# dsshim0125/s2p

Measured on AMD Instinct MI355X. Metric: G+D train-step images/sec at 84x84 bs=64/GPU, higher is better.
Workload: dtype bf16; 1 GPU; configs[2]: full G+D train step (hinge GAN + feature matching + VGG19 perceptual + L1, Adam x2), 84x84 cheetah, netG=s2p, netD=multiscale(2); global_batch=64, per_gpu_batch=64, parallelism=dp1, hip_graph=True, graph_segments=1, streams=overlapped, vgg_weights=seeded stand-in (ImageNet weights unobtainable offline)

## Files before the change

include/s2p_hip.h:

```cpp
#ifndef S2P_HIP_H
#define S2P_HIP_H
#include <stddef.h>
#include <stdint.h>

#ifdef __cplusplus
extern "C" {
#endif
#pragma GCC visibility push(default)

#define S2P_VERSION 125

enum { S2P_F32 = 0, S2P_BF16 = 1 };
enum { S2P_ACT_NONE = 0, S2P_ACT_RELU = 1, S2P_ACT_LRELU = 2, S2P_ACT_TANH = 3, S2P_ACT_SWISH = 4 };
enum { S2P_EPI_STORE = 0,
       S2P_EPI_ADD = 1,
       S2P_EPI_MUL_ACTGRAD = 2   };

typedef struct {
  int32_t dtype;
  int32_t N, H, W, Cin, x_pitch;
  int32_t Ho, Wo, Cout, y_pitch;
  int32_t KH, KW, stride, pad;
  int32_t transposed;
  int32_t reflect;
  int32_t groups;
  int32_t x_gstride, y_gstride;
  int32_t cin_real;
} s2p_conv_desc;

int s2p_version(void);
const char* s2p_last_error(void);

int s2p_conv2d_fwd(const s2p_conv_desc* d, const void* x, const void* w_fwd, const float* bias,
                   const void* aux, void* y, int act, float slope, int epi, void* stream);
int s2p_conv2d_dgrad(const s2p_conv_desc* d, const void* dy, const void* w_bwd,
                     const void* aux, const void* aux2, void* dx, int epi, int aux_act, float slope,
                     void* stream);
size_t s2p_conv2d_fwd_workspace(const s2p_conv_desc* d, int epi);
int s2p_conv2d_fwd_ws(const s2p_conv_desc* d, const void* x, const void* w_fwd, const float* bias,
                      const void* aux, void* y, int act, float slope, int epi, void* workspace,
                      size_t workspace_bytes, void* stream);
size_t s2p_conv2d_dgrad_workspace(const s2p_conv_desc* d);
int s2p_conv2d_dgrad_ws(const s2p_conv_desc* d, const void* dy, const void* w_bwd,
                        const void* aux, const void* aux2, void* dx, int epi, int aux_act, float slope,
                        void* workspace, size_t workspace_bytes, void* stream);
int s2p_conv2d_fwd_mat(const s2p_conv_desc* d, const void* x, const void* w_fwd, const float* bias, const void* aux,
                       void* y, int epi, const void* gb_img, int gb_pitch, const float* gb_st, int gb_st_pitch,
                       int act, float slope, float eps, void* y_mat, int y_mat_pitch, float* stats, void* workspace,
                       size_t workspace_bytes, void* stream);
int s2p_conv2d_dgrad_mat(const s2p_conv_desc* d, const void* dy, const void* w_bwd, void* d_mid, const void* aux, const void* xn,
                         int xn_pitch, const float* stats, const void* gb_img, int gb_pitch, const float* gb_st,
                         int gb_st_pitch, int act, float slope, float eps, float* sums, void* dxn, int dxn_pitch,
                         void* dgb_img, int dgb_pitch, float* dgb_st, int dgb_st_pitch, const void* res, int res_pitch,
                         void* workspace, size_t workspace_bytes, void* stream);
int s2p_conv2d_mat_is_fused(const s2p_conv_desc* d, int dgrad, int has_gb);
enum { S2P_CONV_PATH_THIN = 0, S2P_CONV_PATH_THIN4 = 1, S2P_CONV_PATH_THIN_CIN = 2, S2P_CONV_PATH_THIN_ROWS = 3,
       S2P_CONV_PATH_PLANE = 4, S2P_CONV_PATH_PLANEG = 5, S2P_CONV_PATH_HALO = 6, S2P_CONV_PATH_SPLITK = 7,
       S2P_CONV_PATH_DMA = 8, S2P_CONV_PATH_PHASES = 9, S2P_CONV_PATH_GENERIC = 10 };
enum { S2P_HALO_S9_176_PIPE = 0, S2P_HALO_S9_176 = 1, S2P_HALO_S9_320 = 2, S2P_HALO_R_176 = 3, S2P_HALO_R_320 = 4 };
int s2p_conv2d_path(const s2p_conv_desc* d, int dgrad, int has_workspace);
int s2p_conv2d_wgrad(const s2p_conv_desc* d, const void* x, const void* dy, float* dw, float* db,
                     int cin_real, int cout_real, int64_t dw_gstride, int splitk, void* stream);
size_t s2p_conv2d_wgrad_workspace(const s2p_conv_desc* d, int cin_real, int cout_real);
int s2p_conv2d_wgrad_ws(const s2p_conv_desc* d, const void* x, const void* dy, float* dw, float* db,
                        int cin_real, int cout_real, int64_t dw_gstride, int splitk, void* workspace,
                        size_t workspace_bytes, void* stream);
size_t s2p_conv2d_wgrad_det_workspace(const s2p_conv_desc* d, int cin_real, int cout_real, int splitk);
typedef struct { const void* x; const void* dy; float* dw; float* db; } s2p_wgrad_job;
size_t s2p_conv2d_wgrad_batched_workspace(const s2p_conv_desc* d, int n_jobs, int cin_real, int cout_real);
int s2p_conv2d_wgrad_batched(const s2p_conv_desc* d, const s2p_wgrad_job* jobs, int n_jobs, int cin_real,
                             int cout_real, void* workspace, size_t workspace_bytes, void* stream);
int s2p_reflect_pad_bwd(int dtype, const void* dxp, int N, int H, int W, int C, int pad, void* dx,
                        void* stream);
int s2p_channel_sum(int dtype, const void* dy, int64_t pixels, int C, int pitch, float* db,
                    void* stream);
size_t s2p_channel_sum_workspace(int64_t pixels, int C);
int s2p_channel_sum_ws(int dtype, const void* dy, int64_t pixels, int C, int pitch, float* db, void* workspace,
                       size_t workspace_bytes, void* stream);

int64_t s2p_in_stats_floats(int N, int HW, int C);
int s2p_in_stats(int dtype, const void* x, int N, int HW, int C, int pitch, float eps,
                 float* stats, void* stream);
int s2p_in_apply_fwd(int dtype, const void* x, int N, int HW, int C, int pitch,
                     const float* stats, const void* gb_img, int gb_pitch,
                     const float* gb_st, int gb_st_pitch, int act, float slope, float eps,
                     void* y, int y_pitch, void* stream);
int s2p_in_norm_fwd(int dtype, const void* x, int N, int HW, int C, int pitch, const void* gb_img, int gb_pitch,
                    const float* gb_st, int gb_st_pitch, int act, float slope, float eps, void* y, int y_pitch,
                    float* stats, void* stream);
int64_t s2p_in_bwd_sums_floats(int N, int HW, int C);
int s2p_in_bwd_reduce(int dtype, const void* da, int da_pitch, const void* x, int N, int HW, int C,
                      int pitch, const float* stats, const void* gb_img, int gb_pitch,
                      const float* gb_st, int gb_st_pitch, int act, float slope, float eps,
                      float* sums, void* stream);
int s2p_in_bwd_apply(int dtype, const void* da, int da_pitch, const void* x, int N, int HW, int C,
                     int pitch, const float* stats, const void* gb_img, int gb_pitch,
                     const float* gb_st, int gb_st_pitch, int act, float slope, float eps,
                     const float* sums, void* dx, int dx_pitch, void* dgb_img, int dgb_pitch,
                     float* dgb_st, int dgb_st_pitch, void* stream);

int s2p_posenc_fwd(const float* state, int N, int S, int L, float* out, int out_pitch, void* stream);

int s2p_in_norm_bwd(int dtype, const void* da, int da_pitch, const void* x, int N, int HW, int C, int pitch,
                    const float* stats, const void* gb_img, int gb_pitch, const float* gb_st, int gb_st_pitch,
                    int act, float slope, float eps, float* sums, void* dx, int dx_pitch, void* dgb_img,
                    int dgb_pitch, float* dgb_st, int dgb_st_pitch, void* stream);
int s2p_in_norm_bwd_res(int dtype, const void* da, int da_pitch, const void* x, int N, int HW, int C, int pitch,
                        const float* stats, const void* gb_img, int gb_pitch, const float* gb_st, int gb_st_pitch,
                        int act, float slope, float eps, float* sums, void* dx, int dx_pitch, void* dgb_img,
                        int dgb_pitch, float* dgb_st, int dgb_st_pitch, const void* res, int res_pitch, void* stream);

// ... 114 lines not shown
```

s2p_amd/_lib.py:

```python
import ctypes
import os
import subprocess

import torch

_HERE = os.path.dirname(os.path.abspath(__file__))
_SO = os.path.join(_HERE, "csrc", "libs2p_hip.so")

F32, BF16 = 0, 1
ACT_NONE, ACT_RELU, ACT_LRELU, ACT_TANH, ACT_SWISH = 0, 1, 2, 3, 4
EPI_STORE, EPI_ADD, EPI_MUL_ACTGRAD = 0, 1, 2
(PATH_THIN, PATH_THIN4, PATH_THIN_CIN, PATH_THIN_ROWS, PATH_PLANE, PATH_PLANEG, PATH_HALO, PATH_SPLITK, PATH_DMA, PATH_PHASES,
 PATH_GENERIC) = range(11)
HALO_S9_176_PIPE, HALO_S9_176, HALO_S9_320, HALO_R_176, HALO_R_320 = range(5)

c_int, c_float, c_void_p, c_int64 = ctypes.c_int, ctypes.c_float, ctypes.c_void_p, ctypes.c_int64


class ConvDesc(ctypes.Structure):
    _fields_ = [(n, ctypes.c_int32) for n in (
        "dtype", "N", "H", "W", "Cin", "x_pitch", "Ho", "Wo", "Cout", "y_pitch",
        "KH", "KW", "stride", "pad", "transposed", "reflect", "groups", "x_gstride", "y_gstride", "cin_real")]


class L1Job(ctypes.Structure):
    _fields_ = [("a", c_void_p), ("b", c_void_p), ("grad_a", c_void_p), ("count", c_int64), ("scale", c_float),
                ("loss_out", c_void_p)]


class WgradJob(ctypes.Structure):
    _fields_ = [("x", c_void_p), ("dy", c_void_p), ("dw", c_void_p), ("db", c_void_p)]


class PackJob(ctypes.Structure):
    _fields_ = [("src", c_void_p), ("dst_fwd", c_void_p), ("dst_bwd", c_void_p),
                ("R", ctypes.c_int32), ("T", ctypes.c_int32), ("C", ctypes.c_int32),
                ("Cpad", ctypes.c_int32), ("Rrow", ctypes.c_int32), ("r_off", ctypes.c_int32),
                ("dtype", ctypes.c_int32)]


class SnJob(ctypes.Structure):
    _fields_ = [("w", c_void_p), ("u", c_void_p), ("v", c_void_p), ("sigma", c_void_p), ("ws", c_void_p), ("grad", c_void_p),
                ("R", ctypes.c_int32), ("K", ctypes.c_int32)]


_P = c_void_p
_DESC = ctypes.POINTER(ConvDesc)
SIGNATURES = {
    "s2p_version": [],
    "s2p_last_error": [],
    "s2p_conv2d_fwd": [_DESC, _P, _P, _P, _P, _P, c_int, c_float, c_int, _P],
    "s2p_conv2d_dgrad": [_DESC, _P, _P, _P, _P, _P, c_int, c_int, c_float, _P],
    "s2p_conv2d_fwd_workspace": [_DESC, c_int],
    "s2p_conv2d_fwd_ws": [_DESC, _P, _P, _P, _P, _P, c_int, c_float, c_int, _P, ctypes.c_size_t, _P],
    "s2p_conv2d_fwd_mat": [_DESC, _P, _P, _P, _P, _P, c_int, _P, c_int, _P, c_int, c_int, c_float, c_float, _P, c_int, _P, _P,
                           ctypes.c_size_t, _P],
    "s2p_conv2d_dgrad_mat": [_DESC, _P, _P, _P, _P, _P, c_int, _P, _P, c_int, _P, c_int, c_int, c_float, c_float, _P, _P, c_int, _P, c_int,
                             _P, c_int, _P, c_int, _P, ctypes.c_size_t, _P],
    "s2p_conv2d_mat_is_fused": [_DESC, c_int, c_int],
    "s2p_conv2d_path": [_DESC, c_int, c_int],
    "s2p_conv2d_dgrad_workspace": [_DESC],
    "s2p_conv2d_dgrad_ws": [_DESC, _P, _P, _P, _P, _P, c_int, c_int, c_float, _P, ctypes.c_size_t, _P],
    "s2p_conv2d_wgrad": [_DESC, _P, _P, _P, _P, c_int, c_int, c_int64, c_int, _P],
    "s2p_conv2d_wgrad_workspace": [_DESC, c_int, c_int],
    "s2p_conv2d_wgrad_det_workspace": [_DESC, c_int, c_int, c_int],
    "s2p_channel_sum_workspace": [c_int64, c_int],
# ... 136 lines not shown
```

s2p_amd/csrc/conv_igemm.hip:

```cpp
#include "s2p_common.h"
#include "conv_plane.h"
#include "conv_planeg.h"
#include <type_traits>
#include <vector>

#define MAX_TAPS 64

constexpr int PHASE_TAPS = 16, MAX_PHASES = 4;
struct GatherArgs {
  const void* x; const void* w; const float* bias; const void* aux; const void* aux2; void* y;
  int M, Hi, Wi, Qh, Qw;
  int Cin, x_pitch, x_gstride;
  int Cout, Cst, y_pitch, y_gstride;
  int Ho, Wo;
  int istride, ostride, oy0, ox0;
  int T, Ktot, w_row;
  long long w_gstride;
  int reflect, act, epi, gact;
  float slope, gslope;
  int npix_tiles, nco_tiles;
  int halo_lo, halo_hi;
  int diag;
  int splitk, ksteps;
  float* part; int psplit, psteps, part_m;
  void* ws; size_t ws_bytes;
  unsigned x_bytes, w_bytes;
  int tap[MAX_TAPS];
  int nphase, phase_fast;
  struct Phase { int Qh, Qw, M, oy0, ox0, T, Ktot, npix_tiles; int tap[PHASE_TAPS]; } ph[MAX_PHASES];
};

template <typename T> struct Mma;
template <> struct Mma<__bf16> { static constexpr int BK = 32; };
template <> struct Mma<float> { static constexpr int BK = 16; };

template <typename T, int BCO, int BPIX, int TCO, int TPIX>
__device__ __forceinline__ void conv_epilogue(const GatherArgs& a, f32x16 (&acc)[TCO][TPIX], char* smem, const int* rowoff,
                                              int g, int co_base, int wco0, int wpix0, int r, int h, int tid) {
  constexpr int CE = DT<T>::CE;
  constexpr int ERS = BCO * (int)sizeof(T) + 16;
  const float* bias = (a.bias && (blockIdx.z == 0 || a.nphase > 0)) ? a.bias + (size_t)g * a.Cout : nullptr;
  const bool act_generic = (a.act == S2P_ACT_TANH || a.act == S2P_ACT_SWISH);
  const float ns = a.act == S2P_ACT_RELU ? 0.f : (a.act == S2P_ACT_LRELU ? a.slope : 1.f);
  if (bias) {
    const __amdgpu_buffer_rsrc_t brs = __builtin_amdgcn_make_buffer_rsrc((void*)bias, 0, a.Cout * 4, 0x00020000);
#pragma unroll
    for (int i = 0; i < TCO; ++i)
#pragma unroll
      for (int q4 = 0; q4 < 4; ++q4) {
        const int co = co_base + wco0 + 32 * i + 8 * q4 + 4 * h;
        float bv[4];
#pragma unroll
        for (int e = 0; e < 4; ++e) bv[e] = __builtin_bit_cast(float, __builtin_amdgcn_raw_buffer_load_b32(brs, co * 4, e * 4, 0));
#pragma unroll
        for (int j = 0; j < TPIX; ++j)
// ... 500 lines not shown
    if (m >= a.M) break;
    Chunk<T> c;
    float wv[8];
#pragma unroll
    for (int e = 0; e < 8; ++e) {
      const float t = v[e][i];
      float w = lrelu_ns(t, ns);
      if (act_generic) w = a.act == S2P_ACT_TANH ? tanhf(t) : t / (1.f + expf(-t));
      wv[e] = w;
    }
    c.pack(wv);
    const size_t go = (size_t)m * a.y_pitch + co0;
    if (a.epi != S2P_EPI_STORE) {
      Chunk<T> x, x2;
      x.raw = (u32x4){0u, 0u, 0u, 0u}; x2.raw = (u32x4){0u, 0u, 0u, 0u};
      if (full) {
        x.raw = *(const u32x4*)(aux + go);
        if (aux2) x2.raw = *(const u32x4*)(aux2 + go);
      } else {
        for (int e = 0; e < 8; ++e) if (co0 + e < a.Cst) {
          x.set(e, to_f32(aux[go + e]));
          if (aux2) x2.set(e, to_f32(aux2[go + e]));
        }
      }
#pragma unroll
      for (int e = 0; e < 8; ++e) {
        const float xv = x.get(e);
        const float f = g_tanh ? 1.f - xv * xv : (xv > 0.f ? 1.f : gneg);
        wv[e] = epi_add ? c.get(e) + xv : (c.get(e) + x2.get(e)) * f;
      }
      c.pack(wv);
    }
    if (full) *(u32x4*)(y + go) = c.raw;
    else for (int e = 0; e < 8; ++e) if (co0 + e < a.Cst) y[go + e] = from_f32<T>(c.get(e));
  }
}

struct ConvSwitches {
  int no_dma = s2p_env_set("S2P_NO_LDS_DMA");
  int diag = s2p_env_int("S2P_DIAG", 0);
  int no_halo = s2p_env_set("S2P_NO_HALO");
  int no_split = s2p_env_set("S2P_NO_CONV_SPLITK");
  int split_min_steps = s2p_env_int("S2P_SPLIT_MIN_STEPS", 16);
  int split_max_wg = s2p_env_int("S2P_SPLIT_MAX_WG", 160);
  int no_plane = s2p_env_set("S2P_NO_PLANE");
  int halo_extra_lds = s2p_env_int("S2P_HALO_EXTRA_LDS", 0);
  int no_static_taps = s2p_env_set("S2P_NO_STATIC_TAPS");
  int halo_pipe = s2p_env_set("S2P_NO_HALO_PIPE") ? 0 : 1;
  int no_merge = s2p_env_set("S2P_NO_PHASE_MERGE") || s2p_env_set("S2P_NO_LDS_DMA");
  int no_thin_cin = s2p_env_set("S2P_NO_THIN_CIN");
  static bool no_planeg() { return S2P_DIAG_SWITCH(0); }
  static bool no_planeg_3x3() { return S2P_DIAG_SWITCH(2); }
  static bool no_thin4() { return S2P_DIAG_SWITCH(3); }
  static bool no_phase_fast() { return S2P_DIAG_SWITCH(10); }
};
static const ConvSwitches& conv_switches() { static const ConvSwitches sw; return sw; }

static int conv_split_plan(int nwg, int nk) {
  const int min_steps = conv_switches().split_min_steps, max_wg = conv_switches().split_max_wg;
  if (nwg > max_wg || nk < 2 * min_steps) return 1;
  int S = 384 / nwg;
  if (S > nk / min_steps) S = nk / min_steps;
  if (S > 16) S = 16;
  return S < 2 ? 1 : S;
}

template <int NPOS_CAP, bool DBUF>
struct HaloTile {
  static constexpr int BCO = 128, BPIX = 128, WPIX = 2, TCO = 2, TPIX = 2;
  static constexpr int BK = 64, RS = 128;
  static constexpr int WSTAGE = BCO * RS;
  static constexpr int HALO = (NPOS_CAP + 1) * RS;
  static constexpr int ERS = BCO * 2 + 16, EPI = BPIX * ERS;
  static constexpr int NHB = DBUF ? 2 : 1;
  static constexpr int MAIN0 = NHB * HALO + 2 * WSTAGE + 1024;
  static constexpr int MAIN = MAIN0 > EPI ? MAIN0 : EPI;
  static constexpr int NHP = (NPOS_CAP / 8 + 3) / 4;

  char* hbase; char* wbase; char* zrow; int* rowoff;
  int tid, lane, wave, r, h, g, lrow, pc;
  int co_base, pix_base, wco0, wpix0, swr, npos, nslab;
  unsigned w_byte[4], h_byte[NHP];
  unsigned long long vmask[TPIX];
  __amdgpu_buffer_rsrc_t xr, wr;

  __device__ __forceinline__ void setup(const GatherArgs& a, char* smem) {
    rowoff = (int*)(smem + MAIN);
    hbase = smem; wbase = smem + NHB * HALO; zrow = smem + NHB * HALO + 2 * WSTAGE;
    tid = threadIdx.x; lane = tid & 63; r = lane & 31; h = lane >> 5; g = blockIdx.y;
    wave = __builtin_amdgcn_readfirstlane(tid >> 6);
    tile_of_block<BCO, BPIX>(blockIdx.x, a.npix_tiles * a.nco_tiles, a.nco_tiles, co_base, pix_base);
    if (tid < BPIX) rowoff[tid] = pix_base + tid < a.M ? pix_base + tid : -1;
    if (tid < 64) *(u32x4*)(zrow + tid * 16) = (u32x4){0u, 0u, 0u, 0u};
    if (tid < 8 * NHB) *(u32x4*)(hbase + (tid >> 3) * HALO + NPOS_CAP * RS + (tid & 7) * 16) = (u32x4){0u, 0u, 0u, 0u};
    xr = conv_x_rsrc(a, g); wr = conv_w_rsrc(a, g);

    lrow = lane >> 3; pc = lane & 7;
#pragma unroll
    for (int i = 0; i < 4; ++i) w_byte[i] = w_row_dma_byte(a, co_base, (4 * i + wave) * 8 + lrow, pc);
    npos = BPIX + a.halo_lo + a.halo_hi;
#pragma unroll
    for (int i = 0; i < NHP; ++i) h_byte[i] = halo_dma_byte(a, (4 * i + wave) * 8 + lrow);
    wco0 = (wave / WPIX) * (TCO * 32);
    wpix0 = (wave % WPIX) * (TPIX * 32);
    const PixelSplit split(a.Qh, a.Qw);
#pragma unroll
// ... 252 lines not shown
  constexpr bool PIPELINED = TS > 0 && PIPE && DBUF;
  __shared__ __attribute__((aligned(1024))) char smem[HT::MAIN + HT::BPIX * 4];
  unsigned long long tl0 = 0, tl1 = 0, tl2 = 0, st_c0 = 0, st_r0 = 0;
  if (S2P_DIAGV(a) == 9) tl0 = __builtin_amdgcn_s_memrealtime();
  HT t;
  t.setup(a, smem);
  f32x16 acc[HT::TCO][HT::TPIX];
  clear_acc(acc);
  if (S2P_DIAGV(a) == 5) return;
  auto loop_start = [&]() {
    if (S2P_DIAGV(a) == 3) return false;
    if (S2P_DIAGV(a) == 8) { st_c0 = __builtin_amdgcn_s_memtime(); st_r0 = __builtin_amdgcn_s_memrealtime(); }
    if (PIPELINED && S2P_DIAGV(a) == 9) tl1 = __builtin_amdgcn_s_memrealtime();
    return true;
  };
  bool done;
  if constexpr (TS > 0) {
    const HaloStaticTaps<TS> tp(a, t);
    if constexpr (PIPELINED) done = halo_loop_pipelined(a, t, tp, acc, loop_start);
    else done = halo_loop_static(a, t, tp, acc, loop_start);
  } else {
    done = halo_loop_runtime(a, t, acc, loop_start);
  }
  if (!done) return;
  if (S2P_DIAGV(a) == 8) {
    const unsigned long long c1 = __builtin_amdgcn_s_memtime(), r1 = __builtin_amdgcn_s_memrealtime();
    if (t.tid == 0 && t.g == 0) {
      unsigned long long* o = (unsigned long long*)a.y + (size_t)blockIdx.x * 2;
      o[0] = c1 - st_c0; o[1] = r1 - st_r0;
    }
    if (acc[0][0][0] == 12345.678f) ((float*)a.y)[7] = acc[1][1][3] + acc[0][1][2] + acc[1][0][1];
    return;
  }
  if constexpr (PIPELINED) {
    asm volatile("s_waitcnt lgkmcnt(0)" ::: "memory");
    __syncthreads();
  }
  if (S2P_DIAGV(a) == 4) { if (acc[0][0][0] == 12345.678f) ((float*)a.y)[0] = acc[1][1][3] + acc[0][1][2] + acc[1][0][1]; return; }
  if (PIPELINED && S2P_DIAGV(a) == 9) {
    tl2 = __builtin_amdgcn_s_memrealtime();
    GatherArgs b = a; b.aux = nullptr;
    conv_epilogue<__bf16, HT::BCO, HT::BPIX, HT::TCO, HT::TPIX>(b, acc, smem, t.rowoff, t.g, t.co_base, t.wco0, t.wpix0, t.r, t.h, t.tid);
    asm volatile("s_waitcnt vmcnt(0)" ::: "memory");
    __syncthreads();
    if (t.tid == 0 && t.g == 0 && a.aux) {
      unsigned long long* o = (unsigned long long*)a.aux + (size_t)blockIdx.x * 4;
      o[0] = tl0; o[1] = tl1; o[2] = tl2; o[3] = __builtin_amdgcn_s_memrealtime();
    }
    return;
  }
  conv_epilogue<__bf16, HT::BCO, HT::BPIX, HT::TCO, HT::TPIX>(a, acc, smem, t.rowoff, t.g, t.co_base, t.wco0, t.wpix0, t.r, t.h, t.tid);
}

enum class ConvPath { Thin, Thin4, ThinCin, ThinRows, Plane, PlaneG, Halo, SplitK, Dma, Phases, Generic };
static_assert((int)ConvPath::Halo == S2P_CONV_PATH_HALO && (int)ConvPath::Generic == S2P_CONV_PATH_GENERIC, "ids of s2p_conv2d_path");
enum class HaloKind { S9_176_PIPE, S9_176, S9_320, R_176, R_320 };

struct ConvOperands {
  const void* x; const void* w; const float* bias; const void* aux; const void* aux2; void* y;
  int act; float slope; int epi, gact; float gslope;
};
struct NormWant { bool any, gb, bwd; };
struct ScratchAvail { bool any; size_t bytes; };
static const ScratchAvail SCRATCH_UNLIMITED{true, ~(size_t)0};
struct Scratch { void* ws; size_t bytes; };

struct GatherChoice {
  ConvPath path = ConvPath::Generic;
  bool fused = false;
  size_t ws_bytes = 0;
  int bco = 128;
  HaloKind halo = HaloKind::R_320;
  PlaneArgs plane;
  PlaneGArgs planeg;
};
struct GatherItem { GatherArgs a; GatherChoice c; };
struct ConvPlan {
  ConvPath path = ConvPath::Generic;
  bool fused = false;
  size_t ws_bytes = 0;
  int cout_pad = 0;
  std::vector<GatherItem> items;
  void add(const GatherItem& it) {
    if (items.empty()) path = it.c.path;
    if (it.c.ws_bytes > ws_bytes) ws_bytes = it.c.ws_bytes;
    items.push_back(it);
    fused = items.size() == 1 && it.c.fused;
  }
};

template <typename P>
static void copy_conv_fields(P& p, const GatherArgs& a) {
  p.x = a.x; p.w = a.w; p.bias = a.bias; p.aux = a.aux; p.aux2 = a.aux2; p.y = a.y;
  p.Cin = a.Cin; p.x_pitch = a.x_pitch; p.x_gstride = a.x_gstride;
  p.Cout = a.Cout; p.Cst = a.Cst; p.y_pitch = a.y_pitch; p.y_gstride = a.y_gstride;
  p.w_row = a.w_row; p.w_gstride = a.w_gstride;
  p.act = a.act; p.epi = a.epi; p.gact = a.gact; p.slope = a.slope; p.gslope = a.gslope;
  p.x_bytes = a.x_bytes; p.w_bytes = a.w_bytes;
}

static void plan_fast(GatherArgs& a, GatherChoice& c, int groups, const NormWant& want, const ScratchAvail& sc) {
  const ConvSwitches& sw = conv_switches();
  a.npix_tiles = cdiv(a.M, 128);
  a.nco_tiles = cdiv(a.Cst, c.bco);
  a.diag = sw.diag;
  const int nwg = a.npix_tiles * a.nco_tiles;
  const bool whole = a.ostride == 1 && a.oy0 == 0 && a.ox0 == 0 && a.Qh == a.Ho && a.Qw == a.Wo;
  const bool planes = whole && a.M % (a.Qh * a.Qw) == 0;
  int S = 1;
  if (!sw.no_split && groups == 1 && whole && sc.any) S = conv_split_plan(nwg, a.Ktot / 64);
  if (!sw.no_plane && a.T == 9 && a.istride == 1 && planes && a.Qh == a.Hi && a.Qw == a.Wi) {
    PlaneArgs& p = c.plane;
    bool ok = true;
    for (int t = 0; t < 9; ++t) p.wt[t] = -1;
    for (int t = 0; t < 9 && ok; ++t) {
      const int dy = (int)(signed char)(a.tap[t] & 0xff), dx = (int)(signed char)((a.tap[t] >> 8) & 0xff);
      if (dy < -1 || dy > 1 || dx < -1 || dx > 1 || p.wt[(dy + 1) * 3 + dx + 1] >= 0) ok = false;
      else p.wt[(dy + 1) * 3 + dx + 1] = a.tap[t] >> 16;
    }
    copy_conv_fields(p, a);
    p.N = a.M / (a.Qh * a.Qw); p.H = a.Qh; p.W = a.Qw;
    if (ok && s2p_conv_plane_applicable(p)) {
      c.path = ConvPath::Plane;
      c.fused = want.any && groups == 1 && a.act == S2P_ACT_NONE && a.epi != S2P_EPI_MUL_ACTGRAD && (!want.bwd || a.epi == S2P_EPI_STORE);
      return;
    }
  }
  if (!sw.no_plane && !sw.no_planeg() && !(a.T == 9 && sw.no_planeg_3x3()) && groups == 1 && planes && !a.reflect) {
    PlaneGProblem pr{a.M / (a.Qh * a.Qw), a.Hi, a.Wi, a.Ho, a.Wo, a.Cin, a.Cout, a.Cst, a.x_pitch, a.y_pitch, a.istride, a.T, a.tap, want.any};
    PlaneGArgs& p = c.planeg;
    if (s2p_conv_planeg_setup(pr, p)) {
      copy_conv_fields(p, a);
      p.N = pr.N;
      c.path = ConvPath::PlaneG;
      c.fused = want.any && p.nbands == 1 && p.gimg == 1 && !want.gb && a.act == S2P_ACT_NONE && a.epi != S2P_EPI_MUL_ACTGRAD;
      return;
    }
  }
  if (c.bco == 128 && S <= 1 && !sw.no_halo && a.istride == 1 && a.ostride == 1 && a.Qh == a.Hi && a.Qw == a.Wi &&
      a.Ho == a.Qh && a.Wo == a.Qw && a.T >= 4) {
    int lo = 0, hi = 0;
    for (int t = 0; t < a.T; ++t) {
      int off = (int)(signed char)(a.tap[t] & 0xff) * a.Wi + (int)(signed char)((a.tap[t] >> 8) & 0xff);
      if (-off > lo) lo = -off;
      if (off > hi) hi = off;
    }
    const int npos = 128 + lo + hi;
    const bool s9 = a.T == 9 && !sw.no_static_taps;
    if (npos <= 320) {
      a.halo_lo = lo; a.halo_hi = hi;
      c.path = ConvPath::Halo;
      if (npos <= 176) c.halo = s9 ? (sw.halo_pipe && a.Cin % 64 == 0 ? HaloKind::S9_176_PIPE : HaloKind::S9_176) : HaloKind::R_176;
      else c.halo = s9 ? HaloKind::S9_320 : HaloKind::R_320;
      return;
    }
  }
  if (S > 1) {
    const int nk = a.Ktot / 64;
    a.psteps = cdiv(nk, S); a.psplit = cdiv(nk, a.psteps);
    a.part_m = a.npix_tiles * 128;
    const size_t need = (size_t)a.psplit * a.Cst * a.part_m * sizeof(float);
    if (a.psplit > 1 && need <= sc.bytes) { c.path = ConvPath::SplitK; c.ws_bytes = need; return; }
    a.psplit = 1;
  }
  c.path = ConvPath::Dma;
}

static GatherItem plan_gather(const GatherArgs& a_in, bool bf16, int groups, long long x_elems, const NormWant& want, const ScratchAvail& sc) {
  GatherItem it{a_in, {}};
  GatherArgs& a = it.a;
  const long long xb = x_elems * 2, wb = (long long)a.Cout * a.w_row * 2;
  if (bf16 && a.Cin % 64 == 0 && !a.reflect && a.T > 0 && xb < (1ll << 31) && wb < (1ll << 31) && a.Cst > 32 && !conv_switches().no_dma) {
    a.x_bytes = (unsigned)xb; a.w_bytes = (unsigned)wb;
    it.c.bco = a.Cst > 64 ? 128 : 64;
    plan_fast(a, it.c, groups, want, sc);
  }
  return it;
}

static int pack_tap(int dy, int dx, int wt) { return (wt << 16) | ((dx & 0xff) << 8) | (dy & 0xff); }

struct Geo {
  int N, Hi, Wi, Ci, xp, xg, Ho, Wo, Co, Cst, yp, yg, KH, KW, stride, pad, reflect, groups;
  long long w_gstride; int w_row;
// ... 147 lines not shown
  return plan_scatter_problem(G, d->dtype == S2P_BF16, op, want, sc, P);
}

template <int BCO>
static int launch_bf16(GatherArgs& a, const GatherChoice& c, int groups, void* ws, hipStream_t st) {
  const int extra_lds = conv_switches().halo_extra_lds;
  dim3 grid(a.npix_tiles * a.nco_tiles, groups);
  switch (c.path) {
    case ConvPath::Halo:
      if constexpr (BCO == 128) {
        switch (c.halo) {
          case HaloKind::S9_176_PIPE: hipLaunchKernelGGL((conv_halo_kernel<176, true, 9, true>), grid, dim3(256), extra_lds, st, a); break;
          case HaloKind::S9_176: hipLaunchKernelGGL((conv_halo_kernel<176, true, 9>), grid, dim3(256), extra_lds, st, a); break;
          case HaloKind::S9_320: hipLaunchKernelGGL((conv_halo_kernel<320, false, 9>), grid, dim3(256), 0, st, a); break;
          case HaloKind::R_176: hipLaunchKernelGGL((conv_halo_kernel<176, true>), grid, dim3(256), extra_lds, st, a); break;
          case HaloKind::R_320: hipLaunchKernelGGL((conv_halo_kernel<320, false>), grid, dim3(256), 0, st, a); break;
        }
        S2P_CHECK_LAUNCH("conv_halo_kernel");
      }
      return 0;
    case ConvPath::SplitK: {
      a.part = (float*)ws;
      grid.z = a.psplit;
      hipLaunchKernelGGL((conv_dma_kernel<BCO, 128, 2, 2>), grid, dim3(256), 0, st, a);
      S2P_CHECK_LAUNCH("conv_dma_kernel(split)");
      const long long n = (long long)(a.part_m / 4) * ((a.Cst + 7) / 8);
      hipLaunchKernelGGL(conv_part_reduce_kernel, dim3(cdiv(n, 64)), dim3(64), 0, st, a);
      S2P_CHECK_LAUNCH("conv_part_reduce_kernel");
      return 0;
    }
    default:
      hipLaunchKernelGGL((conv_dma_kernel<BCO, 128, 2, 2>), grid, dim3(256), 0, st, a);
      S2P_CHECK_LAUNCH("conv_dma_kernel");
      return 0;
  }
}

template <typename T>
static int launch_generic(GatherArgs& a, int groups, hipStream_t st) {
  if (a.Cst > 64) return launch_cfg<T, 128, 128, 2, 2>(a, groups, st);
  if (a.Cst > 32) return launch_cfg<T, 64, 128, 2, 2>(a, groups, st);
  return launch_cfg<T, 32, 256, 1, 4>(a, groups, st);
}

static int launch_item(GatherItem& it, bool bf16, int groups, const PlaneNorm* mat, void* ws, hipStream_t st) {
  if (!bf16) return launch_generic<float>(it.a, groups, st);
  switch (it.c.path) {
    case ConvPath::Plane:
      if (it.c.fused) it.c.plane.nm = *mat;
      return s2p_conv_plane_launch(it.c.plane, groups, st);
    case ConvPath::PlaneG:
      if (it.c.fused) it.c.planeg.nm = *mat;
      return s2p_conv_planeg_launch(it.c.planeg, groups, st);
    case ConvPath::Phases: {
      GatherArgs& a = it.a;
      int max_npt = 0;
      for (int i = 0; i < a.nphase; ++i) if (a.ph[i].npix_tiles > max_npt) max_npt = a.ph[i].npix_tiles;
      const dim3 grid = a.phase_fast ? dim3(((max_npt * a.nco_tiles + 7) / 8) * 8 * a.nphase, groups, 1) : dim3(max_npt * a.nco_tiles, groups, a.nphase);
      if (it.c.bco == 128) hipLaunchKernelGGL((conv_dma_kernel<128, 128, 2, 2>), grid, dim3(256), 0, st, a);
      else hipLaunchKernelGGL((conv_dma_kernel<64, 128, 2, 2>), grid, dim3(256), 0, st, a);
      S2P_CHECK_LAUNCH("conv_dma_kernel(phases)");
      return 0;
    }
    case ConvPath::Generic: break;
    default: return it.c.bco == 128 ? launch_bf16<128>(it.a, it.c, groups, ws, st) : launch_bf16<64>(it.a, it.c, groups, ws, st);
  }
  return launch_generic<__bf16>(it.a, groups, st);
}
static int launch_items(ConvPlan& P, bool bf16, int groups, const PlaneNorm* mat, const Scratch& sc, hipStream_t st) {
  for (GatherItem& it : P.items) {
    const int rc = launch_item(it, bf16, groups, mat, sc.ws, st);
    if (rc) return rc;
  }
  return 0;
}

static int conv_fwd_impl(const s2p_conv_desc* d, const ConvOperands& op, const PlaneNorm* mat, bool* fused, const Scratch& sc, void* stream) {
  S2P_CHECK_SLOPE("s2p_conv2d_fwd", op.act, op.slope);
  if (mat) S2P_CHECK_SLOPE("s2p_conv2d_fwd_mat", mat->n_act, mat->n_slope);
  ConvPlan P;
  int rc = conv_plan_fwd(d, op, NormWant{mat != nullptr, mat && mat->gb, false}, ScratchAvail{sc.ws != nullptr, sc.bytes}, P);
  if (rc) return rc;
  if (!op.x || !op.w || (!op.y && !mat)) S2P_FAIL(-1, "s2p_conv2d_fwd: null pointer");
  if (op.epi != S2P_EPI_STORE && !op.aux) S2P_FAIL(-1, "s2p_conv2d_fwd: epi needs aux");
  if (!op.y && !P.fused) S2P_FAIL(-1, "s2p_conv2d_fwd_mat: y == NULL needs the fused launch (s2p_conv2d_mat_is_fused)");
  if (fused) *fused = P.fused;
  hipStream_t st = (hipStream_t)stream;
  switch (P.path) {
    case ConvPath::Thin: return s2p_thin_fwd(d, op.x, op.w, op.bias, op.y, op.act, op.slope, st);
    case ConvPath::Thin4: return s2p_thin4_fwd(d, op.x, op.w, op.bias, op.y, op.act, op.slope, sc.ws, sc.bytes, st);
    case ConvPath::ThinCin: return s2p_thin_cin_fwd(d, op.x, op.w, op.bias, op.y, op.act, op.slope, st);
    default: return launch_items(P, d->dtype == S2P_BF16, d->groups, mat, sc, st);
  }
}

extern "C" int s2p_conv2d_fwd(const s2p_conv_desc* d, const void* x, const void* w_fwd, const float* bias,
                              const void* aux, void* y, int act, float slope, int epi, void* stream) {
  return conv_fwd_impl(d, ConvOperands{x, w_fwd, bias, aux, nullptr, y, act, slope, epi, 0, 0.f}, nullptr, nullptr, Scratch{nullptr, 0}, stream);
}
extern "C" int s2p_conv2d_fwd_ws(const s2p_conv_desc* d, const void* x, const void* w_fwd, const float* bias,
                                 const void* aux, void* y, int act, float slope, int epi, void* workspace,
                                 size_t workspace_bytes, void* stream) {
  return conv_fwd_impl(d, ConvOperands{x, w_fwd, bias, aux, nullptr, y, act, slope, epi, 0, 0.f}, nullptr, nullptr,
                       Scratch{workspace, workspace_bytes}, stream);
}
extern "C" int s2p_conv2d_fwd_mat(const s2p_conv_desc* d, const void* x, const void* w_fwd, const float* bias, const void* aux,
// ... 95 lines not shown
```

Before: 7649 images/sec.

## Add persistent streaming 3x3 conv kernel with LDS ring buffer for Cin=64

Adds a new conv path for 3x3 stride-1 convolutions with 64 input channels that would otherwise take the multi-band PlaneG path without fused norm. Each workgroup is persistent per CU and per 64-channel output slice. It keeps all 9 taps of weights resident in LDS and streams input pixels through a padded-row ring buffer, refilling the next tile inside the MFMA K loop. This is meant to remove the repeated weight and halo reloads of the banded PlaneG kernel and to overlap loads with compute. The trade-off is one workgroup per CU at 256 threads, which lowers occupancy and may leave CUs idle when there are few tiles.

```diff
diff --git a/include/s2p_hip.h b/include/s2p_hip.h
--- a/include/s2p_hip.h
+++ b/include/s2p_hip.h
@@ -56,7 +56,7 @@
 int s2p_conv2d_mat_is_fused(const s2p_conv_desc* d, int dgrad, int has_gb);
 enum { S2P_CONV_PATH_THIN = 0, S2P_CONV_PATH_THIN4 = 1, S2P_CONV_PATH_THIN_CIN = 2, S2P_CONV_PATH_THIN_ROWS = 3,
        S2P_CONV_PATH_PLANE = 4, S2P_CONV_PATH_PLANEG = 5, S2P_CONV_PATH_HALO = 6, S2P_CONV_PATH_SPLITK = 7,
-       S2P_CONV_PATH_DMA = 8, S2P_CONV_PATH_PHASES = 9, S2P_CONV_PATH_GENERIC = 10 };
+       S2P_CONV_PATH_DMA = 8, S2P_CONV_PATH_PHASES = 9, S2P_CONV_PATH_GENERIC = 10, S2P_CONV_PATH_STREAM = 11 };
 enum { S2P_HALO_S9_176_PIPE = 0, S2P_HALO_S9_176 = 1, S2P_HALO_S9_320 = 2, S2P_HALO_R_176 = 3, S2P_HALO_R_320 = 4 };
 int s2p_conv2d_path(const s2p_conv_desc* d, int dgrad, int has_workspace);
 int s2p_conv2d_wgrad(const s2p_conv_desc* d, const void* x, const void* dy, float* dw, float* db,
diff --git a/s2p_amd/_lib.py b/s2p_amd/_lib.py
--- a/s2p_amd/_lib.py
+++ b/s2p_amd/_lib.py
@@ -11,7 +11,7 @@
 ACT_NONE, ACT_RELU, ACT_LRELU, ACT_TANH, ACT_SWISH = 0, 1, 2, 3, 4
 EPI_STORE, EPI_ADD, EPI_MUL_ACTGRAD = 0, 1, 2
 (PATH_THIN, PATH_THIN4, PATH_THIN_CIN, PATH_THIN_ROWS, PATH_PLANE, PATH_PLANEG, PATH_HALO, PATH_SPLITK, PATH_DMA, PATH_PHASES,
- PATH_GENERIC) = range(11)
+ PATH_GENERIC, PATH_STREAM) = range(12)
 HALO_S9_176_PIPE, HALO_S9_176, HALO_S9_320, HALO_R_176, HALO_R_320 = range(5)
 
 c_int, c_float, c_void_p, c_int64 = ctypes.c_int, ctypes.c_float, ctypes.c_void_p, ctypes.c_int64
diff --git a/s2p_amd/csrc/conv_igemm.hip b/s2p_amd/csrc/conv_igemm.hip
--- a/s2p_amd/csrc/conv_igemm.hip
+++ b/s2p_amd/csrc/conv_igemm.hip
@@ -1,6 +1,7 @@
 #include "s2p_common.h"
 #include "conv_plane.h"
 #include "conv_planeg.h"
+#include "conv_stream.h"
 #include <type_traits>
 #include <vector>
 
@@ -607,6 +608,7 @@
   static bool no_planeg() { return S2P_DIAG_SWITCH(0); }
   static bool no_planeg_3x3() { return S2P_DIAG_SWITCH(2); }
   static bool no_thin4() { return S2P_DIAG_SWITCH(3); }
+  static bool no_stream() { return S2P_DIAG_SWITCH(21); }
   static bool no_phase_fast() { return S2P_DIAG_SWITCH(10); }
 };
 static const ConvSwitches& conv_switches() { static const ConvSwitches sw; return sw; }
@@ -965,8 +967,9 @@
   conv_epilogue<__bf16, HT::BCO, HT::BPIX, HT::TCO, HT::TPIX>(a, acc, smem, t.rowoff, t.g, t.co_base, t.wco0, t.wpix0, t.r, t.h, t.tid);
 }
 
-enum class ConvPath { Thin, Thin4, ThinCin, ThinRows, Plane, PlaneG, Halo, SplitK, Dma, Phases, Generic };
-static_assert((int)ConvPath::Halo == S2P_CONV_PATH_HALO && (int)ConvPath::Generic == S2P_CONV_PATH_GENERIC, "ids of s2p_conv2d_path");
+enum class ConvPath { Thin, Thin4, ThinCin, ThinRows, Plane, PlaneG, Halo, SplitK, Dma, Phases, Generic, Stream };
+static_assert((int)ConvPath::Halo == S2P_CONV_PATH_HALO && (int)ConvPath::Generic == S2P_CONV_PATH_GENERIC && (int)ConvPath::Stream == S2P_CONV_PATH_STREAM,
+              "ids of s2p_conv2d_path");
 enum class HaloKind { S9_176_PIPE, S9_176, S9_320, R_176, R_320 };
 
 struct ConvOperands {
@@ -986,6 +989,7 @@
   HaloKind halo = HaloKind::R_320;
   PlaneArgs plane;
   PlaneGArgs planeg;
+  StreamArgs stream;
 };
 struct GatherItem { GatherArgs a; GatherChoice c; };
 struct ConvPlan {
@@ -1043,6 +1047,18 @@
     PlaneGProblem pr{a.M / (a.Qh * a.Qw), a.Hi, a.Wi, a.Ho, a.Wo, a.Cin, a.Cout, a.Cst, a.x_pitch, a.y_pitch, a.istride, a.T, a.tap, want.any};
     PlaneGArgs& p = c.planeg;
     if (s2p_conv_planeg_setup(pr, p)) {
+      if (p.nbands > 1 && a.Cin == 64 && !want.any && !sw.no_stream()) {
+        const StreamProblem sp{pr.N, a.Hi, a.Wi, a.Ho, a.Wo, a.Cin, a.Cout, a.Cst, a.x_pitch, a.y_pitch, a.istride, a.T, a.tap};
+        StreamArgs& s = c.stream;
+        if (s2p_conv_stream_setup(sp, s)) {
+          s.x = a.x; s.w = a.w; s.bias = a.bias; s.aux = a.aux; s.aux2 = a.aux2; s.y = a.y;
+          s.x_pitch = a.x_pitch; s.Cout = a.Cout; s.y_pitch = a.y_pitch; s.w_row = a.w_row;
+          s.act = a.act; s.epi = a.epi; s.gact = a.gact; s.slope = a.slope; s.gslope = a.gslope;
+          s.x_bytes = a.x_bytes; s.w_bytes = a.w_bytes;
+          c.path = ConvPath::Stream;
+          return;
+        }
+      }
       copy_conv_fields(p, a);
       p.N = pr.N;
       c.path = ConvPath::PlaneG;
@@ -1296,6 +1312,8 @@
     case ConvPath::PlaneG:
       if (it.c.fused) it.c.planeg.nm = *mat;
       return s2p_conv_planeg_launch(it.c.planeg, groups, st);
+    case ConvPath::Stream:
+      return s2p_conv_stream_launch(it.c.stream, st);
     case ConvPath::Phases: {
       GatherArgs& a = it.a;
       int max_npt = 0;
diff --git a/s2p_amd/csrc/conv_stream.h b/s2p_amd/csrc/conv_stream.h
--- /dev/null
+++ b/s2p_amd/csrc/conv_stream.h
@@ -0,0 +1,23 @@
+#pragma once
+#include <hip/hip_runtime.h>
+
+struct StreamArgs {
+  const void* x; const void* w; const float* bias; const void* aux; const void* aux2; void* y;
+  int N, H, W;
+  int Hp, Wp;
+  int total;
+  int hA;
+  int x_pitch, Cout, y_pitch, w_row;
+  int wt[9];
+  int act, epi, gact;
+  float slope, gslope;
+  unsigned x_bytes, w_bytes;
+  int ntiles, tpw, nranges, nco;
+};
+
+struct StreamProblem {
+  int N, Hi, Wi, Ho, Wo, Cin, Cout, Cst, x_pitch, y_pitch, istride, T;
+  const int* tap;
+};
+bool s2p_conv_stream_setup(const StreamProblem& p, StreamArgs& a);
+int s2p_conv_stream_launch(const StreamArgs& a, hipStream_t st);
diff --git a/s2p_amd/csrc/conv_stream.hip b/s2p_amd/csrc/conv_stream.hip
--- /dev/null
+++ b/s2p_amd/csrc/conv_stream.hip
@@ -0,0 +1,185 @@
+#include "s2p_common.h"
+#include "conv_stream.h"
+#include "conv_plane_epi.h"
+
+namespace {
+constexpr int CS_PB = 3;
+constexpr int CS_T = 4 * CS_PB * 16;
+constexpr int CS_HMAX = 96;
+constexpr int CS_CAP = 2 * CS_T + 2 * CS_HMAX;
+constexpr int CS_WBYTES = 9 * 64 * 128;
+constexpr int CS_NPC = CS_T / 8 / 4;
+static_assert(CS_CAP % 8 == 0 && CS_T % 32 == 0 && CS_NPC <= 18, "pieces are 8 ring positions; the refill goes out in the K loop's steps");
+
+__device__ __forceinline__ int cs_wrap(int x) { return x >= CS_CAP ? x - CS_CAP : x; }
+
+struct CsRows {
+  char* ring; int base;
+  __device__ __forceinline__ char* operator()(int px, int c) const { return ring + cs_wrap(base + px) * 128 + ((c ^ (px & 7)) << 4); }
+};
+}
+
+__global__ __launch_bounds__(256, 1) void conv_stream_kernel(const StreamArgs a) {
+  typedef __bf16 T;
+  constexpr int PB = CS_PB;
+  __shared__ __attribute__((aligned(1024))) char smem[CS_WBYTES + CS_CAP * 128];
+  char* const wbase = smem;
+  char* const ring = smem + CS_WBYTES;
+
+  const int tid = threadIdx.x, lane = tid & 63;
+  const int wave = __builtin_amdgcn_readfirstlane(tid >> 6);
+  const int q = lane >> 4, l15 = lane & 15;
+  const int cs = (int)(blockIdx.x >> 3) % a.nco, rg = ((int)(blockIdx.x >> 3) / a.nco) * 8 + (int)(blockIdx.x & 7);
+  const int t0 = rg * a.tpw;
+  const int t1 = t0 + a.tpw < a.ntiles ? t0 + a.tpw : a.ntiles;
+  if (t0 >= t1) return;
+  const int co_base = cs * 64;
+
+  const i32x4 xrs = s2p_make_rsrc(a.x, a.x_bytes);
+  const i32x4 wrs = s2p_make_rsrc(a.w, a.w_bytes);
+  const unsigned w_lds = __builtin_amdgcn_readfirstlane(s2p_lds_addr(wbase));
+  const unsigned r_lds = __builtin_amdgcn_readfirstlane(s2p_lds_addr(ring));
+  const int OOB = (int)0x80000000u;
+  const int Wp = a.Wp, Hp = a.Hp, hA = a.hA;
+
+  const float rwp = 1.0f / (float)Wp, rhp = 1.0f / (float)Hp;
+  auto split = [&](int p, int& n, int& r, int& c) {
+    int row = (int)(((float)p + 0.5f) * rwp);
+    c = p - row * Wp;
+    if (c < 0) { --row; c += Wp; }
+    if (c >= Wp) { ++row; c -= Wp; }
+    n = (int)(((float)row + 0.5f) * rhp);
+    r = row - n * Hp;
+    if (r < 0) { --n; r += Hp; }
+    if (r >= Hp) { ++n; r -= Hp; }
+    return p >= 0 && p < a.total && c < a.W && r < a.H;
+  };
+  auto issue_in = [&](int pstart, int ri) {
+    int n, r, c;
+    const bool ok = split(pstart + (lane >> 3), n, r, c);
+    const int v = ok ? (int)((((unsigned)(n * a.H + r) * a.W + c) * a.x_pitch) * 2u + (unsigned)(((lane & 7) ^ (lane >> 3)) * 16)) : OOB;
+    s2p_dma16(xrs, r_lds + (unsigned)ri * 128u, v);
+  };
+
+  {
+    const int col = lane >> 3;
+#pragma unroll
+    for (int k = 0; k < 18; ++k) {
+      const int pi = wave + 4 * k, tap = pi >> 3, co = co_base + (pi & 7) * 8 + col;
+      const int v = co < a.Cout ? (int)((unsigned)co * a.w_row * 2u + (unsigned)(((lane & 7) ^ col) * 16)) : OOB;
+      s2p_dma16_so(wrs, w_lds + (unsigned)pi * 1024u, v, a.wt[tap] * 128);
+    }
+  }
+  int base = (int)(((long long)t0 * CS_T) % CS_CAP);
+  {
+    const int np0 = (CS_T + 2 * hA) >> 3;
+    for (int m = wave; m < np0; m += 4) issue_in(t0 * CS_T - hA + 8 * m, cs_wrap(base + 8 * m));
+  }
+  const int aA0 = l15 * 128 + ((q ^ (l15 & 7)) << 4), aA1 = aA0 ^ 64;
+  const float* bias = a.bias ? a.bias + co_base : nullptr;
+  T* const y = (T*)a.y;
+  const PeOut eo(a.aux, a.aux2, 0, a.epi, a.gact, a.gslope);
+  S2P_WAIT_VMCNT(0);
+
+  for (int t = t0; t < t1; ++t) {
+    asm volatile("s_waitcnt lgkmcnt(0)" ::: "memory");
+    __builtin_amdgcn_s_barrier();
+    asm volatile("" ::: "memory");
+    __builtin_amdgcn_sched_barrier(0);
+    const int tp0 = t * CS_T;
+    const bool refill = t + 1 < t1;
+    int bB[PB][9];
+#pragma unroll
+    for (int j = 0; j < PB; ++j) {
+      const int i = (wave * PB + j) * 16 + l15;
+#pragma unroll
+      for (int k = 0; k < 9; ++k) {
+        const int x = cs_wrap(base + hA + i + (k / 3 - 1) * Wp + (k % 3 - 1));
+        bB[j][k] = x * 128 + ((q ^ (x & 7)) << 4);
+      }
+    }
+    f32x4 acc[4][PB];
+#pragma unroll
+    for (int i = 0; i < 4; ++i)
+#pragma unroll
+      for (int j = 0; j < PB; ++j) acc[i][j] = (f32x4){0.f, 0.f, 0.f, 0.f};
+
+    auto rd = [&](auto sc, bf16x8 (&fa)[4], bf16x8 (&fb)[PB]) {
+      constexpr int s = decltype(sc)::value, tap = s >> 1, ks = s & 1;
+#pragma unroll
+      for (int i = 0; i < 4; ++i) fa[i] = *(const bf16x8*)(wbase + tap * 8192 + i * 2048 + (ks ? aA1 : aA0));
+#pragma unroll
+      for (int j = 0; j < PB; ++j) fb[j] = *(const bf16x8*)(ring + (bB[j][tap] ^ (ks * 64)));
+    };
+    bf16x8 fa[4], fb[PB];
+    rd(std::integral_constant<int, 0>{}, fa, fb);
+    s2p_static_for<0, 18>([&](auto sc) {
+      constexpr int s = decltype(sc)::value;
+      bf16x8 na[4], nb[PB];
+      if constexpr (s + 1 < 18) rd(std::integral_constant<int, s + 1>{}, na, nb);
+      if constexpr (s < CS_NPC) {
+        if (refill) { const int m = wave + 4 * s; issue_in(tp0 + CS_T + hA + 8 * m, cs_wrap(base + CS_T + 2 * hA + 8 * m)); }
+      }
+#pragma unroll
+      for (int j = 0; j < PB; ++j)
+#pragma unroll
+        for (int i = 0; i < 4; ++i) acc[i][j] = __builtin_amdgcn_mfma_f32_16x16x32_bf16(fa[i], fb[j], acc[i][j], 0, 0, 0);
+      if constexpr (s + 1 < 18) {
+#pragma unroll
+        for (int i = 0; i < 4; ++i) fa[i] = na[i];
+#pragma unroll
+        for (int j = 0; j < PB; ++j) fb[j] = nb[j];
+      }
+    });
+    S2P_WAIT_VMCNT(0);
+    asm volatile("s_waitcnt lgkmcnt(0)" ::: "memory");
+    __builtin_amdgcn_s_barrier();
+    asm volatile("" ::: "memory");
+    __builtin_amdgcn_sched_barrier(0);
+
+    const CsRows srow{ring, base};
+    pe_stage_out<PB, 4, 0>(acc, bias, a.act, a.slope, wave, q, l15, srow);
+#pragma unroll
+    for (int k = 0; k < 2 * PB; ++k) {
+      const int px = wave * (PB * 16) + k * 8 + (lane >> 3), ch = lane & 7;
+      int n, r, c;
+      if (split(tp0 + px, n, r, c)) {
+        const size_t go = ((size_t)(n * a.H + r) * a.W + c) * a.y_pitch + co_base + ch * 8;
+        *(u32x4*)(y + go) = pe_out_chunk(eo, srow, px, ch, go).raw;
+      }
+    }
+    base = cs_wrap(base + CS_T);
+  }
+}
+
+bool s2p_conv_stream_setup(const StreamProblem& p, StreamArgs& a) {
+  if (p.Cin != 64 || p.Cout % 64 || p.Cst != p.Cout || p.x_pitch % 8 || p.y_pitch % 8 || p.istride != 1 || p.T != 9) return false;
+  if (p.Ho != p.Hi || p.Wo != p.Wi || p.Hi < 1 || p.Wi < 1 || p.N < 1) return false;
+  for (int k = 0; k < 9; ++k) a.wt[k] = -1;
+  for (int t = 0; t < 9; ++t) {
+    const int dy = (int)(signed char)(p.tap[t] & 0xff), dx = (int)(signed char)((p.tap[t] >> 8) & 0xff);
+    if (dy < -1 || dy > 1 || dx < -1 || dx > 1 || a.wt[(dy + 1) * 3 + dx + 1] >= 0) return false;
+    a.wt[(dy + 1) * 3 + dx + 1] = p.tap[t] >> 16;
+  }
+  a.N = p.N; a.H = p.Hi; a.W = p.Wi; a.Hp = p.Hi + 1; a.Wp = p.Wi + 1;
+  a.hA = (a.Wp + 1 + 7) & ~7;
+  if (a.hA > CS_HMAX) return false;
+  const long long total = (long long)p.N * a.Hp * a.Wp;
+  if (total > (1ll << 22)) return false;
+  a.total = (int)total;
+  a.ntiles = (a.total + CS_T - 1) / CS_T;
+  a.nco = p.Cout / 64;
+  a.tpw = 0; a.nranges = 0;
+  return true;
+}
+
+int s2p_conv_stream_launch(const StreamArgs& a_in, hipStream_t st) {
+  StreamArgs a = a_in;
+  int nr = s2p_num_cus() / a.nco;
+  if (nr < 1) nr = 1;
+  a.tpw = (a.ntiles + nr - 1) / nr;
+  a.nranges = ((a.ntiles + a.tpw - 1) / a.tpw + 7) & ~7;
+  hipLaunchKernelGGL(conv_stream_kernel, dim3(a.nranges * a.nco), dim3(256), 0, st, a);
+  S2P_CHECK_LAUNCH("conv_stream_kernel");
+  return 0;
+}
```

Result: no change. 7594 images/sec (-0.7%).
